# Itseez/opencv

Measured on AMD Instinct MI355X. Metric: Mpix/s per GPU (4K CV_8U Gaussian5x5) + achieved HBM GB/s vs roofline, 1/2/4/8 GPUs, higher is better.
Workload: dtype u8; 1 GPU; cv::GaussianBlur 5x5 sigma=0 BORDER_REFLECT_101 on 3840x2160 CV_8UC1, 9216 device-resident frames per GPU per step (152.9 GB of HBM: one pass = 18 launches of 512 frames); frames_per_gpu=9216, frames_per_launch=512, ranks=1, collective=none (1 GPU)

## Files before the change

### opencv_amd/csrc/smooth.hip

```cpp
#include "rt.h"
#include "gausskernel.h"
#include "seproll.h"
#include "seplong.h"
#include "sepmx.h"
#include <cstring>
#include <cstdlib>

using namespace mi355;

namespace {

struct FixedTaps { uint16_t kx[33]; uint16_t ky[33]; int nx, ny; };

__global__ __launch_bounds__(256) void k_sepfixed_generic(
    const uchar* __restrict__ src, size_t sstep, size_t sframe,
    uchar* __restrict__ dst, size_t dstep, size_t dframe,
    int W, int H, int cn, int mL, int mT, int mR, int mB, int border, FixedTaps t)
{
    const int b = blockIdx.x * 64 + (threadIdx.x & 63);
    const int y = blockIdx.y * 4 + (threadIdx.x >> 6);
    if (b >= W * cn || y >= H) return;
    src += (size_t)blockIdx.z * sframe;
    dst += (size_t)blockIdx.z * dframe;
    const int x = b / cn, c = b - x * cn;
    const int fullW = mL + W + mR, fullH = mT + H + mB;
    const int rx = t.nx / 2, ry = t.ny / 2;
    uint32_t acc = 0;
    for (int j = 0; j < t.ny; j++) {
        int yy = mi355_borderInterpolate(y + mT + j - ry, fullH, border);
        if (yy < 0) continue;
        const uchar* row = src + (ptrdiff_t)(yy - mT) * (ptrdiff_t)sstep;
        uint32_t h = 0;
        for (int i = 0; i < t.nx; i++) {
            int xx = mi355_borderInterpolate(x + mL + i - rx, fullW, border);
            if (xx < 0) continue;
            h += (uint32_t)t.kx[i] * row[(ptrdiff_t)(xx - mL) * cn + c];
        }
        h = h > 0xFFFFu ? 0xFFFFu : h;
        uint64_t a = (uint64_t)acc + (uint64_t)t.ky[j] * h;
        acc = a > 0xFFFFFFFFull ? 0xFFFFFFFFu : (uint32_t)a;
    }
    uint32_t r = (uint32_t)(((uint64_t)acc + 0x8000u) >> 16);
    dst[(size_t)y * dstep + b] = (uchar)(r > 255 ? 255 : r);
}

constexpr int floordiv2(int a) { return a >= 0 ? a / 2 : -((-a + 1) / 2); }
constexpr int mod2(int a) { return ((a % 2) + 2) % 2; }

template <int Q, int S, int HD>
__device__ __forceinline__ uint32_t pairAt(const uint32_t* E, const uint32_t* O, int k)
{
    constexpr int q2 = mod2(Q + S);
    constexpr int f = floordiv2(Q + S);
    const uint32_t* P = q2 ? O : E;
    if constexpr (mod2(f) == 0) {
        return P[k + f / 2 + HD];
    } else {
        constexpr int lo = floordiv2(f - 1) + 0;
        return __builtin_amdgcn_alignbit(P[k + lo + 1 + HD], P[k + lo + HD], 16);
    }
}

template <int HD> struct RawRow {
    uint4 m;
    uint32_t hl[HD];
    uint32_t hr[HD];
};

template <int KS, int CN> struct RollCfg {
    static constexpr int R = KS / 2;
    static constexpr int HB = R * CN;
    static constexpr int HD = (HB + 3) / 4;
};

template <int KS, int CN>
__device__ __forceinline__ void loadRow(RawRow<RollCfg<KS, CN>::HD>& r, const uchar* __restrict__ src, size_t sstep,
                                        int yy, int W, int H, int c, int nchunks, int lane, int border)
{
    constexpr int HD = RollCfg<KS, CN>::HD, HB = RollCfg<KS, CN>::HB;
    r.m = make_uint4(0, 0, 0, 0);
#pragma unroll
    for (int d = 0; d < HD; d++) { r.hl[d] = 0; r.hr[d] = 0; }
    const int ry = mi355_borderInterpolate(yy, H, border);
    if (ry < 0 || c >= nchunks) return;
    const uchar* row = src + (size_t)ry * sstep;
    r.m = *reinterpret_cast<const uint4*>(row + 16 * (size_t)c);
    if (lane == 0) {
        if (c > 0) {
#pragma unroll
            for (int d = 0; d < HD; d++) r.hl[d] = *reinterpret_cast<const uint32_t*>(row + 16 * (size_t)c - 4 * (HD - d));
        } else {
#pragma unroll
            for (int t = -HB; t < 0; t++) {
                const int px = (t - (CN - 1)) / CN;
                const int ch = t - px * CN;
                const int sp = mi355_borderInterpolate(px, W, border);
                const uint32_t v = sp < 0 ? 0u : row[sp * CN + ch];
                r.hl[(4 * HD + t) >> 2] |= v << (8 * ((4 * HD + t) & 3));
            }
        }
    }
    if (c == nchunks - 1) {
#pragma unroll
        for (int t = 0; t < HB; t++) {
            const int px = W + t / CN, ch = t % CN;
            const int sp = mi355_borderInterpolate(px, W, border);
            const uint32_t v = sp < 0 ? 0u : row[sp * CN + ch];
            r.hr[t >> 2] |= v << (8 * (t & 3));
        }
    } else if (lane == 63) {
#pragma unroll
        for (int d = 0; d < HD; d++) r.hr[d] = *reinterpret_cast<const uint32_t*>(row + 16 * (size_t)c + 16 + 4 * d);
    }
}

template <int KS, int CN>
__device__ __forceinline__ void hfilter(uint32_t (&Hrow)[8], const RawRow<RollCfg<KS, CN>::HD>& r, int c, int nchunks, int lane)
{
    constexpr int HD = RollCfg<KS, CN>::HD;
    constexpr int NW = 4 + 2 * HD;
    uint32_t X[NW];
    const uint32_t mv[4] = {r.m.x, r.m.y, r.m.z, r.m.w};
#pragma unroll
    for (int d = 0; d < HD; d++) {
        uint32_t l = __shfl_up(mv[4 - HD + d], 1);
        uint32_t rr = __shfl_down(mv[d], 1);
        X[d] = (lane == 0) ? r.hl[d] : l;
        X[HD + 4 + d] = (lane == 63 || c == nchunks - 1) ? r.hr[d] : rr;
    }
#pragma unroll
    for (int d = 0; d < 4; d++) X[HD + d] = mv[d];
    uint32_t E[NW], O[NW];
#pragma unroll
    for (int d = 0; d < NW; d++) {
        E[d] = __builtin_amdgcn_perm(0u, X[d], 0x0c020c00u);
        O[d] = __builtin_amdgcn_perm(0u, X[d], 0x0c030c01u);
    }
#pragma unroll
    for (int k = 0; k < 4; k++) {
        if constexpr (KS == 5) {
            {   uint32_t a = pairAt<0, -2 * CN, HD>(E, O, k) + pairAt<0, 2 * CN, HD>(E, O, k);
                uint32_t b = pairAt<0, -CN, HD>(E, O, k) + pairAt<0, CN, HD>(E, O, k);
                uint32_t m = pairAt<0, 0, HD>(E, O, k);
                Hrow[k] = a + (b << 2) + (m << 1) + (m << 2); }
            {   uint32_t a = pairAt<1, -2 * CN, HD>(E, O, k) + pairAt<1, 2 * CN, HD>(E, O, k);
                uint32_t b = pairAt<1, -CN, HD>(E, O, k) + pairAt<1, CN, HD>(E, O, k);
                uint32_t m = pairAt<1, 0, HD>(E, O, k);
                Hrow[4 + k] = a + (b << 2) + (m << 1) + (m << 2); }
        } else {
            Hrow[k]     = pairAt<0, -CN, HD>(E, O, k) + pairAt<0, CN, HD>(E, O, k) + (pairAt<0, 0, HD>(E, O, k) << 1);
            Hrow[4 + k] = pairAt<1, -CN, HD>(E, O, k) + pairAt<1, CN, HD>(E, O, k) + (pairAt<1, 0, HD>(E, O, k) << 1);
        }
    }
}

template <int KS, int CN>
__global__ __launch_bounds__(256) void k_binomial_roll(
    const uchar* __restrict__ src, size_t sstep, size_t sframe,
    uchar* __restrict__ dst, size_t dstep, size_t dframe,
    int W, int H, int nchunks, int segRows, int border)
{
    constexpr int R = KS / 2, HD = RollCfg<KS, CN>::HD;
    const int lane = threadIdx.x & 63;
    const int c = (blockIdx.x * 4 + (threadIdx.x >> 6)) * 64 + lane;
    const int y0 = blockIdx.y * segRows;
    const int y1 = min(H, y0 + segRows);
    src += (size_t)blockIdx.z * sframe;
    dst += (size_t)blockIdx.z * dframe;
    const bool active = c < nchunks;

    uint32_t Hw[KS][8];
    {
        RawRow<HD> pre[KS - 1];
#pragma unroll
        for (int i = 0; i < KS - 1; i++) loadRow<KS, CN>(pre[i], src, sstep, y0 - R + i, W, H, c, nchunks, lane, border);
#pragma unroll
        for (int i = 0; i < KS - 1; i++) hfilter<KS, CN>(Hw[i], pre[i], c, nchunks, lane);
    }
    for (int y = y0; y < y1; y += KS) {
        RawRow<HD> raw[KS];
#pragma unroll
        for (int u = 0; u < KS; u++)
            if (y + u < y1) loadRow<KS, CN>(raw[u], src, sstep, y + u + R, W, H, c, nchunks, lane, border);
#pragma unroll
        for (int u = 0; u < KS; u++) {
            if (y + u < y1) {
                hfilter<KS, CN>(Hw[(KS - 1 + u) % KS], raw[u], c, nchunks, lane);
                uint32_t o[4];
                if constexpr (KS == 5) {
                    const uint32_t* h0 = Hw[(u + 0) % 5]; const uint32_t* h1 = Hw[(u + 1) % 5];
                    const uint32_t* h2 = Hw[(u + 2) % 5]; const uint32_t* h3 = Hw[(u + 3) % 5];
                    const uint32_t* h4 = Hw[(u + 4) % 5];
                    uint32_t v[8];
#pragma unroll
                    for (int i = 0; i < 8; i++) {
                        const uint32_t b4 = lshlAdd(h1[i] + h3[i] + h2[i], 2, 0x00800080u);
                        v[i] = h0[i] + h4[i] + lshlAdd(h2[i], 1, b4);
                    }
#pragma unroll
                    for (int k = 0; k < 4; k++) o[k] = __builtin_amdgcn_perm(v[4 + k], v[k], 0x07030501u);
                } else {
                    const uint32_t* h0 = Hw[(u + 0) % 3]; const uint32_t* h1 = Hw[(u + 1) % 3]; const uint32_t* h2 = Hw[(u + 2) % 3];
#pragma unroll
                    for (int k = 0; k < 4; k++) {
                        uint32_t ve = ((h0[k] + h2[k] + (h1[k] << 1) + 0x00080008u) >> 4) & 0x00FF00FFu;
                        uint32_t vo = ((h0[4 + k] + h2[4 + k] + (h1[4 + k] << 1) + 0x00080008u) >> 4) & 0x00FF00FFu;
                        o[k] = ve | (vo << 8);
                    }
                }
                if (active)
                    *reinterpret_cast<uint4*>(dst + (size_t)(y + u) * dstep + 16 * (size_t)c) = make_uint4(o[0], o[1], o[2], o[3]);
            }
        }
    }
}

template <int HD> struct RawRow2 {
    uint4 m;
    uint32_t side[HD];
};

template <int HD> struct EdgeSel {
    uint32_t la[HD], lb[HD], lc[HD];
    uint32_t ra[HD], rb[HD], rc[HD];
};

__device__ __forceinline__ void selSetByte(uint32_t& a, uint32_t& b, uint32_t& c, int j, int idx )
{
    const uint32_t sh = 8u * (uint32_t)j, clr = ~(0xffu << sh);
    uint32_t va = 0x0cu, vb = 0x0cu, vc = 0x0cu;
    if (idx >= 8)      { vb = (uint32_t)(idx - 8); vc = 4u + (uint32_t)j; }
    else if (idx >= 0) { va = (uint32_t)idx;       vc = (uint32_t)j; }
    a = (a & clr) | (va << sh); b = (b & clr) | (vb << sh); c = (c & clr) | (vc << sh);
}

__device__ __forceinline__ uint32_t gather16(const uint4& m, uint32_t a, uint32_t b, uint32_t c)
{
    const uint32_t t1 = __builtin_amdgcn_perm(m.y, m.x, a);
    const uint32_t t2 = __builtin_amdgcn_perm(m.w, m.z, b);
    return __builtin_amdgcn_perm(t2, t1, c);
}

template <int KS, int CN, bool NTL = false>
__device__ __forceinline__ void issueRow(RawRow2<RollCfg<KS, CN>::HD>& r, const uchar* __restrict__ row, int mainOff, int sideOff)
{
    constexpr int HD = RollCfg<KS, CN>::HD;
    if constexpr (NTL) {
        typedef uint32_t u32x4 __attribute__((ext_vector_type(4)));
        u32x4 v = __builtin_nontemporal_load(reinterpret_cast<const u32x4*>(row + mainOff));
        r.m = make_uint4(v.x, v.y, v.z, v.w);
    } else
    r.m = *reinterpret_cast<const uint4*>(row + mainOff);
#pragma unroll
    for (int d = 0; d < HD; d++) r.side[d] = *reinterpret_cast<const uint32_t*>(row + sideOff + 4 * d);
}

template <int KS, int CN, bool EB = true>
__device__ __forceinline__ void hfilter2(uint32_t (&Hrow)[8], const RawRow2<RollCfg<KS, CN>::HD>& r,
                                         bool hasFirst, bool hasLast, bool isLastChunk, const EdgeSel<RollCfg<KS, CN>::HD>& es)
{
    constexpr int HD = RollCfg<KS, CN>::HD;
    constexpr int NW = 4 + 2 * HD;
    uint32_t X[NW];
    const uint32_t mv[4] = {r.m.x, r.m.y, r.m.z, r.m.w};
    uint32_t hl[HD], hr[HD];
#pragma unroll
    for (int d = 0; d < HD; d++) { hl[d] = r.side[d]; hr[d] = r.side[d]; }
    if (hasFirst) {
#pragma unroll
        for (int d = 0; d < HD; d++) { hl[d] = gather16(r.m, es.la[d], es.lb[d], es.lc[d]); if constexpr (EB) asm volatile("" : "+v"(hl[d])); }
    }
    uint32_t hb[HD];
#pragma unroll
    for (int d = 0; d < HD; d++) hb[d] = 0;
    if (hasLast) {
#pragma unroll
        for (int d = 0; d < HD; d++) { hb[d] = gather16(r.m, es.ra[d], es.rb[d], es.rc[d]); if constexpr (EB) asm volatile("" : "+v"(hb[d])); }
    }
#pragma unroll
    for (int d = 0; d < HD; d++) {
        X[d] = __builtin_amdgcn_update_dpp(hl[d], mv[4 - HD + d], 0x138, 0xf, 0xf, false);
        uint32_t rr = __builtin_amdgcn_update_dpp(hr[d], mv[d], 0x130, 0xf, 0xf, false);
        if (hasLast) { rr = isLastChunk ? hb[d] : rr; if constexpr (EB) asm volatile("" : "+v"(rr)); }
        X[HD + 4 + d] = rr;
    }
#pragma unroll
    for (int d = 0; d < 4; d++) X[HD + d] = mv[d];
    uint32_t E[NW], O[NW];
#pragma unroll
    for (int d = 0; d < NW; d++) {
        E[d] = __builtin_amdgcn_perm(0u, X[d], 0x0c020c00u);
        O[d] = __builtin_amdgcn_perm(0u, X[d], 0x0c030c01u);
    }
#pragma unroll
    for (int k = 0; k < 4; k++) {
        if constexpr (KS == 5) {
            {   uint32_t a = pairAt<0, -2 * CN, HD>(E, O, k) + pairAt<0, 2 * CN, HD>(E, O, k);
                uint32_t b = pairAt<0, -CN, HD>(E, O, k) + pairAt<0, CN, HD>(E, O, k);
                uint32_t m = pairAt<0, 0, HD>(E, O, k);
                Hrow[k] = a + (b << 2) + (m << 1) + (m << 2); }
            {   uint32_t a = pairAt<1, -2 * CN, HD>(E, O, k) + pairAt<1, 2 * CN, HD>(E, O, k);
                uint32_t b = pairAt<1, -CN, HD>(E, O, k) + pairAt<1, CN, HD>(E, O, k);
                uint32_t m = pairAt<1, 0, HD>(E, O, k);
                Hrow[4 + k] = a + (b << 2) + (m << 1) + (m << 2); }
        } else {
            Hrow[k]     = pairAt<0, -CN, HD>(E, O, k) + pairAt<0, CN, HD>(E, O, k) + (pairAt<0, 0, HD>(E, O, k) << 1);
            Hrow[4 + k] = pairAt<1, -CN, HD>(E, O, k) + pairAt<1, CN, HD>(E, O, k) + (pairAt<1, 0, HD>(E, O, k) << 1);
        }
    }
}

template <int KS, int CN, bool NT, bool NTL, int WPS, bool EB = true>
__global__ __launch_bounds__(256, WPS) void k_binomial_roll2(
    const uchar* __restrict__ src, size_t sstep, size_t sframe,
    uchar* __restrict__ dst, size_t dstep, size_t dframe,
    int W, int H, int nchunks, int nstrips, int segRows, int nseg, int nframes, int border, int alt)
{
    constexpr int R = KS / 2, HD = RollCfg<KS, CN>::HD, HB = RollCfg<KS, CN>::HB;
    const int lane = threadIdx.x & 63;
    const int wid = __builtin_amdgcn_readfirstlane((int)(blockIdx.x * 4 + (threadIdx.x >> 6)));
    const int strip = wid % nstrips;
    const int t0 = wid / nstrips;
    int seg = t0 % nseg;
    const int frame = t0 / nseg;
    if (frame >= nframes) return;
    int up = 0;
    if (alt) {
        const int G = 1 << alt, span = 8 * G;
        const int g = seg / span, j = seg - g * span;
        if ((g + 1) * span <= nseg) seg = g * span + G * (j & 7) + (j >> 3);
        else if (alt > 1) {
            const int base = g * span, t = seg - base, g2 = t >> 4, j2 = t & 15;
            if (base + (g2 << 4) + 16 <= nseg) seg = base + (g2 << 4) + 2 * (j2 & 7) + (j2 >> 3);
        }
        up = seg & 1;
    }
    const int c = strip * 64 + lane;
    const int y0 = seg * segRows;
    const int y1 = min(H, y0 + segRows);
    src += (size_t)frame * sframe;
    dst += (size_t)frame * dframe;
    const bool active = c < nchunks;
    const bool hasFirst = strip == 0, hasLast = strip == nstrips - 1;
    const bool isLastChunk = c == nchunks - 1;
    const int ce = active ? c : nchunks - 1;
    const int mainOff = 16 * ce;
    const int c0 = strip * 64;
    const int leftOff = c0 > 0 ? 16 * c0 - 4 * HD : 0;
    const int rightOff = c0 + 64 < nchunks ? 16 * (c0 + 64) : 16 * (nchunks - 1);
    const int sideOff = lane < 32 ? leftOff : rightOff;

    EdgeSel<HD> es;
#pragma unroll
    for (int d = 0; d < HD; d++) { es.la[d] = es.lb[d] = es.lc[d] = es.ra[d] = es.rb[d] = es.rc[d] = 0x0c0c0c0cu; }
    if (hasFirst) {
#pragma unroll
        for (int t = 0; t < HB; t++) {
            const int bt = t - HB;
            const int px = (bt - (CN - 1)) / CN;
            const int sp = mi355_borderInterpolate(px, W, border);
            const int pos = 4 * HD - HB + t;
            selSetByte(es.la[pos >> 2], es.lb[pos >> 2], es.lc[pos >> 2], pos & 3, sp < 0 ? -1 : sp * CN + (bt - px * CN));
        }
    }
    if (hasLast) {
#pragma unroll
        for (int t = 0; t < HB; t++) {
            const int sp = mi355_borderInterpolate(W + t / CN, W, border);
            selSetByte(es.ra[t >> 2], es.rb[t >> 2], es.rc[t >> 2], t & 3, sp < 0 ? -1 : sp * CN + (t % CN) - 16 * (nchunks - 1));
        }
    }
    int rowBelow[R], rowAbove[R];
#pragma unroll
    for (int i = 0; i < R; i++) { rowBelow[i] = mi355_borderInterpolate(H + i, H, border); rowAbove[i] = mi355_borderInterpolate(-1 - i, H, border); }
    const int nrows = y1 - y0;
    auto gy = [&](int j) -> int { return up ? y1 - 1 - j : y0 + j; };
    auto rowIdx = [&](int g) -> int {
        int ry = g;
#pragma unroll
        for (int i = 0; i < R; i++) { ry = (g == H + i) ? rowBelow[i] : ry; ry = (g == -1 - i) ? rowAbove[i] : ry; }
        return ry;
    };

    uint32_t Hw[KS][8];
#pragma unroll
    for (int i = 0; i < KS - 1; i++) {
        const int ry = rowIdx(gy(min(i - R, nrows - 1 + R)));
        if (ry < 0) {
#pragma unroll
            for (int j = 0; j < 8; j++) Hw[i][j] = 0;
        } else {
            RawRow2<HD> pre;
            issueRow<KS, CN>(pre, src + (size_t)ry * sstep, mainOff, sideOff);
            hfilter2<KS, CN, EB>(Hw[i], pre, hasFirst, hasLast, isLastChunk, es);
        }
    }
    RawRow2<HD> raw[KS];
    int rvalid[KS];
#pragma unroll
    for (int u = 0; u < KS; u++) {
        const int ry = rowIdx(gy(min(u + R, nrows - 1 + R)));
        rvalid[u] = ry >= 0;
        issueRow<KS, CN, NTL>(raw[u], src + (size_t)max(ry, 0) * sstep, mainOff, sideOff);
    }
    for (int y = 0; y < nrows; y += KS) {
#pragma unroll
        for (int u = 0; u < KS; u++) {
            if (y + u < nrows) {
                uint32_t (&Hn)[8] = Hw[(KS - 1 + u) % KS];
                if (rvalid[u]) hfilter2<KS, CN, EB>(Hn, raw[u], hasFirst, hasLast, isLastChunk, es);
                else {
#pragma unroll
                    for (int j = 0; j < 8; j++) Hn[j] = 0;
                }
                {
                    const int ry = rowIdx(gy(min(y + u + KS + R, nrows - 1 + R)));
                    rvalid[u] = ry >= 0;
                    issueRow<KS, CN, NTL>(raw[u], src + (size_t)max(ry, 0) * sstep, mainOff, sideOff);
                }
                uint32_t o[4];
                if constexpr (KS == 5) {
                    const uint32_t* h0 = Hw[(u + 0) % 5]; const uint32_t* h1 = Hw[(u + 1) % 5];
                    const uint32_t* h2 = Hw[(u + 2) % 5]; const uint32_t* h3 = Hw[(u + 3) % 5];
                    const uint32_t* h4 = Hw[(u + 4) % 5];
                    uint32_t v[8];
#pragma unroll
                    for (int i = 0; i < 8; i++) {
                        if constexpr (EB) {
                            const uint32_t b4 = lshlAdd(h1[i] + h3[i] + h2[i], 2, 0x00800080u);
                            v[i] = h0[i] + h4[i] + lshlAdd(h2[i], 1, b4);
                        } else
                            v[i] = (h0[i] + h4[i]) + ((h1[i] + h3[i]) << 2) + (h2[i] << 1) + (h2[i] << 2) + 0x00800080u;
                    }
#pragma unroll
                    for (int k = 0; k < 4; k++) o[k] = __builtin_amdgcn_perm(v[4 + k], v[k], 0x07030501u);
                } else {
                    const uint32_t* h0 = Hw[(u + 0) % 3]; const uint32_t* h1 = Hw[(u + 1) % 3]; const uint32_t* h2 = Hw[(u + 2) % 3];
#pragma unroll
                    for (int k = 0; k < 4; k++) {
                        uint32_t ve = ((h0[k] + h2[k] + (h1[k] << 1) + 0x00080008u) >> 4) & 0x00FF00FFu;
                        uint32_t vo = ((h0[4 + k] + h2[4 + k] + (h1[4 + k] << 1) + 0x00080008u) >> 4) & 0x00FF00FFu;
                        o[k] = ve | (vo << 8);
                    }
                }
                if (active) {
                    typedef uint32_t u32x4 __attribute__((ext_vector_type(4)));
                    u32x4 ov = {o[0], o[1], o[2], o[3]};
                    u32x4* dp = reinterpret_cast<u32x4*>(dst + (size_t)gy(y + u) * dstep + 16 * (size_t)c);
                    if constexpr (NT) __builtin_nontemporal_store(ov, dp);
                    else *dp = ov;
                }
            }
        }
    }
}

template <bool NT>
__global__ __launch_bounds__(256) void k_copy16(const uint4* __restrict__ s, uint4* __restrict__ d, size_t n16, int perThread)
{
    typedef uint32_t u32x4 __attribute__((ext_vector_type(4)));
    size_t base = ((size_t)blockIdx.x * perThread) * 256 + threadIdx.x;
#pragma unroll 4
    for (int i = 0; i < perThread; i++) {
        size_t j = base + (size_t)i * 256;
        if (j < n16) {
            uint4 v = s[j];
            u32x4 ov = {v.x, v.y, v.z, v.w};
            if constexpr (NT) __builtin_nontemporal_store(ov, reinterpret_cast<u32x4*>(d + j));
            else d[j] = v;
        }
    }
}

template <int UNROLL>
__global__ __launch_bounds__(256) void k_copy_colwalk(const uchar* __restrict__ src, uchar* __restrict__ dst, size_t step, size_t frame,
                                                      int H, int nchunks, int nstrips, int segRows, int nseg, int nframes)
{
    const int lane = threadIdx.x & 63;
    const int wid = __builtin_amdgcn_readfirstlane((int)(blockIdx.x * 4 + (threadIdx.x >> 6)));
    const int strip = wid % nstrips, t0 = wid / nstrips, seg = t0 % nseg, fr = t0 / nseg;
    if (fr >= nframes) return;
    const int c = strip * 64 + lane;
    if (c >= nchunks) return;
    const int y0 = seg * segRows, y1 = min(H, y0 + segRows);
    const uchar* s = src + (size_t)fr * frame + 16 * (size_t)c;
    uchar* d = dst + (size_t)fr * frame + 16 * (size_t)c;
    for (int y = y0; y < y1; y += UNROLL) {
        uint4 v[UNROLL];
#pragma unroll
        for (int u = 0; u < UNROLL; u++) v[u] = *reinterpret_cast<const uint4*>(s + (size_t)min(y + u, y1 - 1) * step);
#pragma unroll
        for (int u = 0; u < UNROLL; u++) if (y + u < y1) *reinterpret_cast<uint4*>(d + (size_t)(y + u) * step) = v[u];
    }
}


bool aligned16(const void* p, size_t step) { return (((uintptr_t)p | step) & 15) == 0; }

int envInt(const char* n, int d) { const char* v = getenv(n); return v ? atoi(v) : d; }

int& tuneSeg() { static int v = envInt("MI355CV_GAUSS_SEG", 0); return v; }
int& tuneVariant() { static int v = envInt("MI355CV_GAUSS_VARIANT", 3); return v; }

int& tuneAlt() { static int v = envInt("MI355CV_GAUSS_ALT", 1); return v; }
int& tuneLaunchWaves() { static int v = envInt("MI355CV_GAUSS_LAUNCH_WAVES", 393216); return v; }

template <int KS, int CN>
void launchRoll2(const uchar* s, size_t ss, size_t sf, uchar* d, size_t ds, size_t df, int nframes, int W, int H, int border, hipStream_t st, int nt)
{
    const int nchunks = W * CN / 16;
    const int nstrips = divUp(nchunks, 64);
    int seg = tuneSeg();
    if (seg <= 0) {
        long long per = (long long)nstrips * nframes;
        long long wantSeg = (2048 + per - 1) / per;
        seg = (int)((H + wantSeg - 1) / wantSeg);
        const int best = 16;
        if (seg > best) seg = best;
        if (seg < KS) seg = KS;
    }
    if (seg > H) seg = H;
    const int nseg = divUp(H, seg);
    const long long perFrame = (long long)nstrips * nseg;
    long long chunk = tuneLaunchWaves() > 0 ? (tuneLaunchWaves() + perFrame - 1) / perFrame : nframes;
    if (chunk < 1) chunk = 1;
    if (chunk > nframes) chunk = nframes;
    const int nlaunch = (int)((nframes + chunk - 1) / chunk);
    noteKernel("k_binomial_roll2<%d,%d,%s,false,%d,%s> grid=%u x256 seg=%d rows alt=%d, %d launch(es) of <= %lld frames", KS, CN, nt >= 1 ? "true" : "false", nt == 3 ? 6 : 4,
               nt == 2 ? "false" : "true", (unsigned)((perFrame * chunk + 3) / 4), seg, tuneAlt(), nlaunch, chunk);
    for (long long f0 = 0; f0 < nframes; f0 += chunk) {
        const int nf = (int)(nframes - f0 < chunk ? nframes - f0 : chunk);
        const uchar* sp = s + (size_t)f0 * sf;
        uchar* dp = d + (size_t)f0 * df;
        dim3 grid((unsigned)((perFrame * nf + 3) / 4));
        if (nt == 3)      hipLaunchKernelGGL((k_binomial_roll2<KS, CN, true, false, 6>), grid, dim3(256), 0, st, sp, ss, sf, dp, ds, df, W, H, nchunks, nstrips, seg, nseg, nf, border, tuneAlt());
        else if (nt == 2) hipLaunchKernelGGL((k_binomial_roll2<KS, CN, true, false, 4, false>), grid, dim3(256), 0, st, sp, ss, sf, dp, ds, df, W, H, nchunks, nstrips, seg, nseg, nf, border, tuneAlt());
        else if (nt == 1) hipLaunchKernelGGL((k_binomial_roll2<KS, CN, true, false, 4>), grid, dim3(256), 0, st, sp, ss, sf, dp, ds, df, W, H, nchunks, nstrips, seg, nseg, nf, border, tuneAlt());
        else              hipLaunchKernelGGL((k_binomial_roll2<KS, CN, false, false, 4>), grid, dim3(256), 0, st, sp, ss, sf, dp, ds, df, W, H, nchunks, nstrips, seg, nseg, nf, border, tuneAlt());
    }
}

template <int KS, int CN>
void launchRoll(const uchar* s, size_t ss, size_t sf, uchar* d, size_t ds, size_t df, int nframes, int W, int H, int border, hipStream_t st)
{
    const int nchunks = W * CN / 16;
    const int gx = divUp(nchunks, 256);
    const int segEnv = tuneSeg();
    int seg;
    if (segEnv > 0) seg = segEnv;
    else {
        long long stripsWaves = (long long)divUp(nchunks, 64) * nframes;
        long long wantSeg = (16384 + stripsWaves - 1) / stripsWaves;
        if (wantSeg < 1) wantSeg = 1;
        seg = (int)((H + wantSeg - 1) / wantSeg);
        if (seg < 4 * KS) seg = 4 * KS;
    }
    seg = divUp(seg, KS) * KS;
    if (seg > H) seg = divUp(H, KS) * KS;
    dim3 grid(gx, divUp(H, seg), nframes);
    hipLaunchKernelGGL((k_binomial_roll<KS, CN>), grid, dim3(256), 0, st, s, ss, sf, d, ds, df, W, H, nchunks, seg, border);
}

bool rollEligible(const uchar* s, size_t ss, size_t sf, const uchar* d, size_t ds, size_t df, int W, int H, int cn, int ks)
{
    if (ks != 3 && ks != 5) return false;
    if (cn < 1 || cn > 4) return false;
    if (!aligned16(s, ss) || !aligned16(d, ds) || (sf & 15) || (df & 15)) return false;
    if ((W * cn) % 16 != 0) return false;
    if (H < 1) return false;
    return true;
}

static int sepmxMinTaps()
{
    static const int v = std::getenv("MI355CV_SEPMX_MIN_TAPS") ? atoi(std::getenv("MI355CV_SEPMX_MIN_TAPS")) : 7;
    return v;
}

int runSmooth(const char* entry, const uchar* src, size_t sstep, size_t sframe, uchar* dst, size_t dstep, size_t dframe,
              int nframes, int W, int H, int cn, int mL, int mT, int mR, int mB,
              const uint16_t* kx, int nx, const uint16_t* ky, int ny, int border, bool binomial)
{
    if (disabled()) return mi355::declined(__func__, __LINE__, "disabled()");
    if (W <= 0 || H <= 0 || nframes <= 0 || cn < 1 || cn > 4) return mi355::declined(__func__, __LINE__, "W <= 0 || H <= 0 || nframes <= 0 || cn < 1 || cn > 4");
    if (nx < 1 || ny < 1 || nx > lim::GAUSS8U_MAX_KSIZE || ny > lim::GAUSS8U_MAX_KSIZE || !(nx & 1) || !(ny & 1)) return mi355::declined(__func__, __LINE__, "nx < 1 || ny < 1 || nx or ny > lim::GAUSS8U_MAX_KSIZE || !(nx & 1) || !(ny & 1)");
    if (border < 0 || border > B_REFLECT_101) return mi355::declined(__func__, __LINE__, "border < 0 || border > B_REFLECT_101");
    Stager stg;
    if (!ensureDevice()) return mi355::declined(__func__, __LINE__, "!ensureDevice()");
    const bool hostSrc = !isDevicePtr(src);
    if (hostSrc && (size_t)W * H < minPixels()) return mi355::declined(__func__, __LINE__, "hostSrc && (size_t)W * H < minPixels()");
    if (!hostSrc && src == dst) return mi355::declined(__func__, __LINE__, "!hostSrc && src == dst");

    size_t dss = 0, dds = 0;
    const size_t rowB = (size_t)W * cn;
    const uchar* dsrc; uchar* ddst;
    if (nframes == 1) {
        const uchar* top = src - (ptrdiff_t)mT * (ptrdiff_t)sstep - (ptrdiff_t)mL * cn;
        const uchar* dtop = stg.in(top, sstep, (size_t)(mL + W + mR) * cn, mT + H + mB, &dss);
        if (!dtop) return mi355::declined(__func__, __LINE__, "!dtop");
        dsrc = dtop + (size_t)mT * dss + (size_t)mL * cn;
        ddst = stg.out(dst, dstep, rowB, H, &dds);
        if (!ddst) return mi355::declined(__func__, __LINE__, "!ddst");
    } else {
        if (hostSrc || !isDevicePtr(dst)) return setError(MI355CV_NOT_IMPLEMENTED, "%s: batch entry needs device-resident frames", entry);
        dsrc = src; ddst = dst; dss = sstep; dds = dstep;
    }
    hipStream_t st = stream();
    const bool noMargins = !(mL | mT | mR | mB);
    if (binomial && noMargins && rollEligible(dsrc, dss, sframe, ddst, dds, dframe, W, H, cn, nx) && nx == ny) {
#define ROLL(KS_, CN_) do { if (tuneVariant() <= 1 || border == B_WRAP || W <= KS_ / 2) launchRoll<KS_, CN_>(dsrc, dss, sframe, ddst, dds, dframe, nframes, W, H, border, st); \
                            else launchRoll2<KS_, CN_>(dsrc, dss, sframe, ddst, dds, dframe, nframes, W, H, border, st, tuneVariant() - 2); } while (0)
        if (nx == 5) { switch (cn) { case 1: ROLL(5, 1); break; case 2: ROLL(5, 2); break; case 3: ROLL(5, 3); break; default: ROLL(5, 4); } }
        else         { switch (cn) { case 1: ROLL(3, 1); break; case 2: ROLL(3, 2); break; case 3: ROLL(3, 3); break; default: ROLL(3, 4); } }
#undef ROLL
    } else if (std::getenv("MI355CV_SMOOTH_GENERIC") == nullptr && std::max(nx, ny) >= sepmxMinTaps() && !(std::getenv("MI355CV_SEPMX") && std::getenv("MI355CV_SEPMX")[0] == '0') &&
               sepmxRun(stg, dsrc, dss, sframe, ddst, dds, dframe, nframes, W, H, cn, mL + W + mR, mT + H + mB, mL, mT, border, kx, nx, nx / 2, ky, ny, ny / 2, st)) {
    } else if (noMargins && std::getenv("MI355CV_SMOOTH_GENERIC") == nullptr &&
               seprollFixedSmooth(dsrc, dss, sframe, ddst, dds, dframe, nframes, W, H, cn, kx, nx, ky, ny, border, st)) {
    } else if (!noMargins && nframes == 1 && std::getenv("MI355CV_SMOOTH_GENERIC") == nullptr && [&] {
                   const Roi roi = {mL + W + mR, mT + H + mB, mL, mT};
                   return seprollFixedSmooth(dsrc, dss, 0, ddst, dds, 0, 1, W, H, cn, kx, nx, ky, ny, border, st, &roi); }()) {
    } else if (std::getenv("MI355CV_SMOOTH_GENERIC") == nullptr && std::max(nx, ny) < sepmxMinTaps() && !(std::getenv("MI355CV_SEPMX") && std::getenv("MI355CV_SEPMX")[0] == '0') &&
               sepmxRun(stg, dsrc, dss, sframe, ddst, dds, dframe, nframes, W, H, cn, mL + W + mR, mT + H + mB, mL, mT, border, kx, nx, nx / 2, ky, ny, ny / 2, st)) {
    } else if (std::getenv("MI355CV_SMOOTH_GENERIC") == nullptr && [&] {
                   unsigned sx = 0, sy = 0;
                   for (int i = 0; i < nx; i++) sx += kx[i];
                   for (int i = 0; i < ny; i++) sy += ky[i];
                   if (sx > 256 || sy > 256) return false;
                   std::vector<int> ix(kx, kx + nx), iy(ky, ky + ny);
                   const SepLongTaps t = {nullptr, nullptr, ix.data(), iy.data(), nx, ny, nx / 2, ny / 2, 3, 0, 0.f, 0};
                   return seplongRun(stg, dsrc, dss, sframe, ddst, dds, dframe, nframes, W, H, cn, MI355CV_8U, MI355CV_8U, mL + W + mR, mT + H + mB, mL, mT, border, t, st); }()) {
    } else {
        if (nx > 33 || ny > 33) return mi355::declined(__func__, __LINE__, "Q8.8 taps that sum beyond 256 with more than 33 of them");
        FixedTaps t;
        t.nx = nx; t.ny = ny;
        for (int i = 0; i < 33; i++) { t.kx[i] = i < nx ? kx[i] : 0; t.ky[i] = i < ny ? ky[i] : 0; }
        dim3 grid(divUp(W * cn, 64), divUp(H, 4), nframes);
        hipLaunchKernelGGL(k_sepfixed_generic, grid, dim3(256), 0, st, dsrc, dss, sframe, ddst, dds, dframe,
                           W, H, cn, mL, mT, mR, mB, border, t);
    }
    return stg.finish(entry);
}

template <int K>
__global__ __launch_bounds__(256) void k_binom16_direct(const uchar* __restrict__ parent, size_t sstep, uchar* __restrict__ dst, size_t dstep, int W, int H, int cn,
                                                        int mL, int mT, int fullW, int fullH, int border)
{
    constexpr int R = K / 2, SH = K == 3 ? 2 : K == 5 ? 4 : K == 7 ? 6 : 8;
    constexpr uint32_t TAP[9] = {K == 3 ? 1u : K == 5 ? 1u : K == 7 ? 2u : 4u, K == 3 ? 2u : K == 5 ? 4u : K == 7 ? 7u : 13u, K == 3 ? 1u : K == 5 ? 6u : K == 7 ? 14u : 30u,
                                 K == 5 ? 4u : K == 7 ? 18u : 51u, K == 5 ? 1u : K == 7 ? 14u : 60u, K == 7 ? 7u : 51u, K == 7 ? 2u : 30u, 13u, 4u};
    const int e = blockIdx.x * 64 + (threadIdx.x & 63), y = blockIdx.y * 4 + (threadIdx.x >> 6);
    if (e >= W * cn || y >= H) return;
    const int x = e / cn, c = e - x * cn;
    int xs[K];
#pragma unroll
    for (int i = 0; i < K; i++) { const int q = mi355_borderInterpolate(x + mL + i - R, fullW, border); xs[i] = q < 0 ? -1 : q * cn + c; }
    uint32_t acc = 0;
#pragma unroll
    for (int j = 0; j < K; j++) {
        const int q = mi355_borderInterpolate(y + mT + j - R, fullH, border);
        if (q < 0) continue;
        const unsigned short* row = reinterpret_cast<const unsigned short*>(parent + (size_t)q * sstep);
        uint32_t h = 0;
#pragma unroll
        for (int i = 0; i < K; i++) h += xs[i] < 0 ? 0u : TAP[i] * (uint32_t)row[xs[i]];
        acc += TAP[j] * h;
    }
    reinterpret_cast<unsigned short*>(dst + (size_t)y * dstep)[e] = (unsigned short)((acc + (1u << (2 * SH - 1))) >> (2 * SH));
}

int runBinom16(const char* entry, const uchar* src, size_t sstep, uchar* dst, size_t dstep, int W, int H, int cn, int mL, int mT, int mR, int mB, int ksize, int border)
{
    if (disabled() || W <= 0 || H <= 0 || cn < 1 || cn > 4 || (ksize != 3 && ksize != 5 && ksize != 7 && ksize != 9) || border < 0 || border > B_REFLECT_101 ||
        mL < 0 || mT < 0 || mR < 0 || mB < 0 || ((sstep | dstep | (uintptr_t)src | (uintptr_t)dst) & 1))
        return mi355::declined(__func__, __LINE__, "disabled() || W <= 0 || H <= 0 || cn < 1 || cn > 4 || ksize not in {3, 5, 7, 9} || border outside CONSTANT .. REFLECT_101 || negative margins || odd pointers / steps");
    Stager stg;
    if (!ensureDevice()) return mi355::declined(__func__, __LINE__, "!ensureDevice()");
    const bool hostSrc = !isDevicePtr(src);
    if (hostSrc && (size_t)W * H < minPixels()) return mi355::declined(__func__, __LINE__, "hostSrc && (size_t)W * H < minPixels()");
    if (!hostSrc && src == dst) return mi355::declined(__func__, __LINE__, "!hostSrc && src == dst");
    size_t dss = 0, dds = 0;
    const size_t esz = (size_t)cn * 2;
    const uchar* top = src - (ptrdiff_t)mT * (ptrdiff_t)sstep - (ptrdiff_t)mL * (ptrdiff_t)esz;
    const uchar* dtop = stg.in(top, sstep, (size_t)(mL + W + mR) * esz, mT + H + mB, &dss);
    if (!dtop) return mi355::declined(__func__, __LINE__, "!dtop");
    const uchar* dsrc = dtop + (size_t)mT * dss + (size_t)mL * esz;
    uchar* ddst = stg.out(dst, dstep, (size_t)W * esz, H, &dds);
    if (!ddst) return mi355::declined(__func__, __LINE__, "!ddst");
    const Roi roi = {mL + W + mR, mT + H + mB, mL, mT};
    if (cn == 1 && (ksize == 3 || ksize == 5) && border != B_WRAP &&
        seprollBinom16(dsrc, dss, 0, ddst, dds, 0, 1, W, H, ksize, border, stream(), (mL | mT | mR | mB) ? &roi : nullptr))
        return stg.finish(entry);
    dim3 grid(divUp(W * cn, 64), divUp(H, 4));
#define B16(K_) hipLaunchKernelGGL(k_binom16_direct<K_>, grid, dim3(256), 0, stream(), dtop, dss, ddst, dds, W, H, cn, mL, mT, mL + W + mR, mT + H + mB, border)
    if (ksize == 3) B16(3); else if (ksize == 5) B16(5); else if (ksize == 7) B16(7); else B16(9);
#undef B16
    noteKernel("k_binom16_direct<%d> grid=%ux%u x256 cn=%d border=%d", ksize, grid.x, grid.y, cn, border);
    return stg.finish(entry);
}

const uint16_t kBinom1[1] = {256};
const uint16_t kBinom3[3] = {64, 128, 64};
const uint16_t kBinom5[5] = {16, 64, 96, 64, 16};
const uint16_t kBinom7[7] = {8, 28, 56, 72, 56, 28, 8};
const uint16_t kBinom9[9] = {4, 13, 30, 51, 60, 51, 30, 13, 4};

const uint16_t* binomTaps(size_t k)
{
    switch (k) { case 1: return kBinom1; case 3: return kBinom3; case 5: return kBinom5; case 7: return kBinom7; case 9: return kBinom9; }
    return nullptr;
}

}

extern "C" {

MI355CV_API int mi355cv_gaussianBlurBinomial(const uchar* src_data, size_t src_step, uchar* dst_data, size_t dst_step,
        int width, int height, int depth, int cn, size_t margin_left, size_t margin_top, size_t margin_right,
        size_t margin_bottom, size_t ksize, int border_type)
{
    mi355::EntryGuard entry_(__func__);
    if (depth == MI355CV_16U)
        return runBinom16("gaussianBlurBinomial", src_data, src_step, dst_data, dst_step, width, height, cn, (int)margin_left, (int)margin_top, (int)margin_right,
                                 (int)margin_bottom, (int)ksize, border_type & ~MI355CV_BORDER_ISOLATED);
    if (depth != MI355CV_8U) return mi355::declined(__func__, __LINE__, "depth != MI355CV_8U");
    const uint16_t* k = binomTaps(ksize);
    if (!k) return mi355::declined(__func__, __LINE__, "!k");
    return runSmooth("gaussianBlurBinomial", src_data, src_step, 0, dst_data, dst_step, 0, 1, width, height, cn,
                     (int)margin_left, (int)margin_top, (int)margin_right, (int)margin_bottom,
                     k, (int)ksize, k, (int)ksize, border_type & ~MI355CV_BORDER_ISOLATED, true);
}

static int gaussBatchFromHost(const uchar* src, size_t sstep, size_t sframe, uchar* dst, size_t dstep, size_t dframe, int nframes, int W, int H, int cn,
                              const uint16_t* k, int ks, int border)
{
    const HostBatch hb = {src, sstep, sframe, (size_t)W * cn, H, dst, dstep, dframe, (size_t)W * cn, H, nframes};
    return runHostBatch("gaussianBlurBinomialBatch", hb, [&](const uchar* s, size_t ss, size_t sf, uchar* d, size_t ds, size_t df, int nf) {
        return runSmooth("gaussianBlurBinomialBatch", s, ss, nf > 1 ? sf : 0, d, ds, nf > 1 ? df : 0, nf, W, H, cn, 0, 0, 0, 0, k, ks, k, ks, border, true);
    });
}

MI355CV_API int mi355cv_gaussianBlurBinomialBatch(const uchar* src_data, size_t src_step, size_t src_frame_stride,
        uchar* dst_data, size_t dst_step, size_t dst_frame_stride, int nframes,
        int width, int height, int depth, int cn, size_t ksize, int border_type)
{
    mi355::EntryGuard entry_(__func__);
    if (depth != MI355CV_8U) return mi355::declined(__func__, __LINE__, "depth != MI355CV_8U");
    const uint16_t* k = binomTaps(ksize);
    if (!k) return mi355::declined(__func__, __LINE__, "!k");
    if (nframes > 1 && width > 0 && height > 0 && cn >= 1 && cn <= 4 && hostBatchEligible(src_data, dst_data, nframes))
        return gaussBatchFromHost(src_data, src_step, src_frame_stride, dst_data, dst_step, dst_frame_stride, nframes, width, height, cn, k, (int)ksize,
                                  border_type & ~MI355CV_BORDER_ISOLATED);
    if (nframes == 1)
        return runSmooth("gaussianBlurBinomialBatch", src_data, src_step, 0, dst_data, dst_step, 0, 1, width, height, cn,
                         0, 0, 0, 0, k, (int)ksize, k, (int)ksize, border_type & ~MI355CV_BORDER_ISOLATED, true);
    return runSmooth("gaussianBlurBinomialBatch", src_data, src_step, src_frame_stride, dst_data, dst_step, dst_frame_stride,
                     nframes, width, height, cn, 0, 0, 0, 0, k, (int)ksize, k, (int)ksize,
                     border_type & ~MI355CV_BORDER_ISOLATED, true);
}

MI355CV_API int mi355cv_gaussianBlur(const uchar* src_data, size_t src_step, uchar* dst_data, size_t dst_step,
        int width, int height, int depth, int cn, size_t margin_left, size_t margin_top, size_t margin_right,
        size_t margin_bottom, size_t ksize_width, size_t ksize_height, double sigmaX, double sigmaY, int border_type)
{
    mi355::EntryGuard entry_(__func__);
    if (depth != MI355CV_8U) {
        if (depth != MI355CV_16U && depth != MI355CV_16S && depth != MI355CV_32F) return mi355::declined(__func__, __LINE__, "depth is none of 8U / 16U / 16S / 32F");
        const int n = (int)ksize_width, m = (int)ksize_height;
        if (n < 1 || m < 1 || n > lim::GAUSS_FLOAT_MAX_KSIZE || m > lim::GAUSS_FLOAT_MAX_KSIZE || !(n & 1) || !(m & 1)) return mi355::declined(__func__, __LINE__, "kernel size outside 1 .. lim::GAUSS_FLOAT_MAX_KSIZE or even");
        if (sigmaY <= 0) sigmaY = sigmaX;
        const double s1 = sigmaX > 0 ? sigmaX : 0, s2 = sigmaY > 0 ? sigmaY : 0;
        std::vector<double> dx, dy;
        if (!gaussianKernelBitExact(n, s1, dx)) return mi355::declined(__func__, __LINE__, "!gaussianKernelBitExact(n, s1, dx)");
        if (m == n && std::fabs(s1 - s2) < 2.220446049250313e-16) dy = dx;
        else if (!gaussianKernelBitExact(m, s2, dy)) return mi355::declined(__func__, __LINE__, "!gaussianKernelBitExact(m, s2, dy)");
        std::vector<float> fx(dx.begin(), dx.end()), fy(dy.begin(), dy.end());
        const int type = MI355CV_MAKETYPE(depth, cn);
        cvhalFilter2D* ctx = nullptr;
        int rc = mi355cv_sepFilterInit(&ctx, type, type, MI355CV_32F, reinterpret_cast<uchar*>(fx.data()), n, reinterpret_cast<uchar*>(fy.data()), m, -1, -1, 0.0, border_type);
        if (rc != MI355CV_OK) return rc;
        rc = mi355cv_sepFilter(ctx, const_cast<uchar*>(src_data), src_step, dst_data, dst_step, width, height, (int)(margin_left + (size_t)width + margin_right),
                               (int)(margin_top + (size_t)height + margin_bottom), (int)margin_left, (int)margin_top);
        (void)mi355cv_sepFilterFree(ctx);
        return rc;
    }
    if (margin_left | margin_top | margin_right | margin_bottom)
        return mi355::setError(MI355CV_NOT_IMPLEMENTED, "gaussianBlur: submatrix with real margins is the reference's sepFilter2D case");
    if (ksize_width > (size_t)lim::GAUSS8U_MAX_KSIZE || ksize_height > (size_t)lim::GAUSS8U_MAX_KSIZE) return mi355::declined(__func__, __LINE__, "ksize_width or ksize_height > lim::GAUSS8U_MAX_KSIZE");
    if (sigmaY <= 0) sigmaY = sigmaX;
    std::vector<int64_t> qx, qy;
    if (!gaussianKernelFixedQ((int)ksize_width, sigmaX > 0 ? sigmaX : 0, 8, qx)) return mi355::declined(__func__, __LINE__, "!gaussianKernelFixedQ((int)ksize_width, sigmaX > 0 ? sigmaX : 0, 8, qx)");
    if (!gaussianKernelFixedQ((int)ksize_height, sigmaY > 0 ? sigmaY : 0, 8, qy)) return mi355::declined(__func__, __LINE__, "!gaussianKernelFixedQ((int)ksize_height, sigmaY > 0 ? sigmaY : 0, 8, qy)");
    uint16_t kx[lim::GAUSS8U_MAX_KSIZE], ky[lim::GAUSS8U_MAX_KSIZE];
    for (size_t i = 0; i < ksize_width; i++) { if (qx[i] < 0 || qx[i] > 65535) return mi355::declined(__func__, __LINE__, "qx[i] < 0 || qx[i] > 65535"); kx[i] = (uint16_t)qx[i]; }
    for (size_t i = 0; i < ksize_height; i++) { if (qy[i] < 0 || qy[i] > 65535) return mi355::declined(__func__, __LINE__, "qy[i] < 0 || qy[i] > 65535"); ky[i] = (uint16_t)qy[i]; }
    bool binom = ksize_width == ksize_height && (ksize_width == 3 || ksize_width == 5);
    if (binom) {
        const uint16_t* b = binomTaps(ksize_width);
        for (size_t i = 0; i < ksize_width; i++) if (kx[i] != b[i] || ky[i] != b[i]) binom = false;
    }
    return runSmooth("gaussianBlur", src_data, src_step, 0, dst_data, dst_step, 0, 1, width, height, cn,
                     (int)margin_left, (int)margin_top, (int)margin_right, (int)margin_bottom,
                     kx, (int)ksize_width, ky, (int)ksize_height, border_type & ~MI355CV_BORDER_ISOLATED, binom);
}

MI355CV_API int mi355cv_gaussianBlurBatch(const uchar* src_data, size_t src_step, size_t src_frame_stride, uchar* dst_data, size_t dst_step, size_t dst_frame_stride,
        int nframes, int width, int height, int depth, int cn, size_t ksize_width, size_t ksize_height, double sigmaX, double sigmaY, int border_type)
{
    mi355::EntryGuard entry_(__func__);
    if (depth != MI355CV_8U) return mi355::declined(__func__, __LINE__, "depth != MI355CV_8U");
    if (nframes < 1 || !(ksize_width & 1) || !(ksize_height & 1) || ksize_width > (size_t)lim::GAUSS8U_MAX_KSIZE || ksize_height > (size_t)lim::GAUSS8U_MAX_KSIZE)
        return mi355::declined(__func__, __LINE__, "nframes < 1 || even kernel size || ksize > lim::GAUSS8U_MAX_KSIZE");
    if (sigmaY <= 0) sigmaY = sigmaX;
    std::vector<int64_t> qx, qy;
    if (!gaussianKernelFixedQ((int)ksize_width, sigmaX > 0 ? sigmaX : 0, 8, qx) || !gaussianKernelFixedQ((int)ksize_height, sigmaY > 0 ? sigmaY : 0, 8, qy))
        return mi355::declined(__func__, __LINE__, "!gaussianKernelFixedQ");
    uint16_t kx[lim::GAUSS8U_MAX_KSIZE], ky[lim::GAUSS8U_MAX_KSIZE];
    for (size_t i = 0; i < ksize_width; i++) { if (qx[i] < 0 || qx[i] > 65535) return mi355::declined(__func__, __LINE__, "qx[i] < 0 || qx[i] > 65535"); kx[i] = (uint16_t)qx[i]; }
    for (size_t i = 0; i < ksize_height; i++) { if (qy[i] < 0 || qy[i] > 65535) return mi355::declined(__func__, __LINE__, "qy[i] < 0 || qy[i] > 65535"); ky[i] = (uint16_t)qy[i]; }
    bool binom = ksize_width == ksize_height && (ksize_width == 3 || ksize_width == 5);
    if (binom) {
        const uint16_t* b = binomTaps(ksize_width);
        for (size_t i = 0; i < ksize_width; i++) if (kx[i] != b[i] || ky[i] != b[i]) binom = false;
    }
    return runSmooth("gaussianBlurBatch", src_data, src_step, nframes > 1 ? src_frame_stride : 0, dst_data, dst_step, nframes > 1 ? dst_frame_stride : 0, nframes, width, height, cn,
                     0, 0, 0, 0, kx, (int)ksize_width, ky, (int)ksize_height, border_type & ~MI355CV_BORDER_ISOLATED, binom);
}

MI355CV_API int mi355cv_setParam(const char* key, int value)
{
    mi355::EntryGuard entry_(__func__);
    if (!key) return -1;
    if (!strcmp(key, "gauss_seg")) { tuneSeg() = value; return 0; }
    if (!strcmp(key, "gauss_variant")) { tuneVariant() = value; return 0; }
    if (!strcmp(key, "gauss_alt")) { tuneAlt() = value; return 0; }
    if (!strcmp(key, "gauss_launch_waves")) { tuneLaunchWaves() = value; return 0; }
    return -1;
}

MI355CV_API int mi355cv_copyProbe(const void* src, void* dst, size_t bytes, int perThread, int nt)
{
    mi355::EntryGuard entry_(__func__);
    if (!ensureDevice() || (bytes & 15) || perThread < 1) return mi355::declined(__func__, __LINE__, "!ensureDevice() || (bytes & 15) || perThread < 1");
    size_t n16 = bytes / 16;
    size_t blocks = (n16 + (size_t)256 * perThread - 1) / ((size_t)256 * perThread);
    if (nt) hipLaunchKernelGGL((k_copy16<true>), dim3((unsigned)blocks), dim3(256), 0, stream(), (const uint4*)src, (uint4*)dst, n16, perThread);
    else    hipLaunchKernelGGL((k_copy16<false>), dim3((unsigned)blocks), dim3(256), 0, stream(), (const uint4*)src, (uint4*)dst, n16, perThread);
    if (hipGetLastError() != hipSuccess) return MI355CV_ERROR_UNKNOWN;
    if (!asyncMode()) (void)hipStreamSynchronize(stream());
    return MI355CV_OK;
}

MI355CV_API int mi355cv_copyProbeColwalk(const void* src, void* dst, int W, int H, int nframes, int segRows, int unroll)
{
    mi355::EntryGuard entry_(__func__);
    if (!ensureDevice() || (W & 15)) return mi355::declined(__func__, __LINE__, "!ensureDevice() || (W & 15)");
    const int nchunks = W / 16, nstrips = divUp(nchunks, 64), nseg = divUp(H, segRows);
    const long long items = (long long)nstrips * nseg * nframes;
    dim3 grid((unsigned)((items + 3) / 4));
    const uchar* s = (const uchar*)src; uchar* d = (uchar*)dst;
    if (unroll == 1) hipLaunchKernelGGL((k_copy_colwalk<1>), grid, dim3(256), 0, stream(), s, d, (size_t)W, (size_t)W * H, H, nchunks, nstrips, segRows, nseg, nframes);
    else if (unroll == 2) hipLaunchKernelGGL((k_copy_colwalk<2>), grid, dim3(256), 0, stream(), s, d, (size_t)W, (size_t)W * H, H, nchunks, nstrips, segRows, nseg, nframes);
    else if (unroll == 5) hipLaunchKernelGGL((k_copy_colwalk<5>), grid, dim3(256), 0, stream(), s, d, (size_t)W, (size_t)W * H, H, nchunks, nstrips, segRows, nseg, nframes);
    else hipLaunchKernelGGL((k_copy_colwalk<10>), grid, dim3(256), 0, stream(), s, d, (size_t)W, (size_t)W * H, H, nchunks, nstrips, segRows, nseg, nframes);
    if (hipGetLastError() != hipSuccess) return MI355CV_ERROR_UNKNOWN;
    if (!asyncMode()) (void)hipStreamSynchronize(stream());
    return MI355CV_OK;
}

MI355CV_API int mi355cv_getGaussianKernelQ(int n, double sigma, int fractionBits, int64_t* taps)
{
    mi355::EntryGuard entry_(__func__);
    std::vector<int64_t> q;
    if (!gaussianKernelFixedQ(n, sigma, fractionBits, q)) return mi355::declined(__func__, __LINE__, "!gaussianKernelFixedQ(n, sigma, fractionBits, q)");
    for (int i = 0; i < n; i++) taps[i] = q[i];
    return MI355CV_OK;
}

MI355CV_API int mi355cv_getGaussianKernel(int n, double sigma, double* taps)
{
    mi355::EntryGuard entry_(__func__);
    std::vector<double> k;
    if (!gaussianKernelBitExact(n, sigma, k)) return mi355::declined(__func__, __LINE__, "!gaussianKernelBitExact(n, sigma, k)");
    for (int i = 0; i < n; i++) taps[i] = k[i];
    return MI355CV_OK;
}

MI355CV_API int mi355cv_sepSmoothFixedU8(const uchar* src_data, size_t src_step, uchar* dst_data, size_t dst_step,
        int width, int height, int cn, size_t margin_left, size_t margin_top, size_t margin_right, size_t margin_bottom,
        const uint16_t* kx, int kxlen, const uint16_t* ky, int kylen, int border_type)
{
    mi355::EntryGuard entry_(__func__);
    if (!kx || !ky) return mi355::declined(__func__, __LINE__, "!kx || !ky");
    bool binom = kxlen == kylen && (kxlen == 3 || kxlen == 5);
    if (binom) {
        const uint16_t* b = binomTaps(kxlen);
        for (int i = 0; i < kxlen; i++) if (kx[i] != b[i] || ky[i] != b[i]) binom = false;
    }
    return runSmooth("sepSmoothFixedU8", src_data, src_step, 0, dst_data, dst_step, 0, 1, width, height, cn,
                     (int)margin_left, (int)margin_top, (int)margin_right, (int)margin_bottom,
                     kx, kxlen, ky, kylen, border_type & ~MI355CV_BORDER_ISOLATED, binom);
}

}
```

Measured before the change: 2.965 million Mpix/s.

## Add RING prologue variant issuing all halo row loads before filtering

```diff
diff --git a/opencv_amd/csrc/smooth.hip b/opencv_amd/csrc/smooth.hip
--- a/opencv_amd/csrc/smooth.hip
+++ b/opencv_amd/csrc/smooth.hip
@@ -310,7 +310,7 @@
     }
 }
 
-template <int KS, int CN, bool NT, bool NTL, int WPS, bool EB = true>
+template <int KS, int CN, bool NT, bool NTL, int WPS, bool EB = true, bool RING = false>
 __global__ __launch_bounds__(256, WPS) void k_binomial_roll2(
     const uchar* __restrict__ src, size_t sstep, size_t sframe,
     uchar* __restrict__ dst, size_t dstep, size_t dframe,
@@ -383,72 +383,114 @@
     };
 
     uint32_t Hw[KS][8];
-#pragma unroll
-    for (int i = 0; i < KS - 1; i++) {
-        const int ry = rowIdx(gy(min(i - R, nrows - 1 + R)));
-        if (ry < 0) {
-#pragma unroll
-            for (int j = 0; j < 8; j++) Hw[i][j] = 0;
-        } else {
-            RawRow2<HD> pre;
-            issueRow<KS, CN>(pre, src + (size_t)ry * sstep, mainOff, sideOff);
-            hfilter2<KS, CN, EB>(Hw[i], pre, hasFirst, hasLast, isLastChunk, es);
-        }
-    }
     RawRow2<HD> raw[KS];
     int rvalid[KS];
-#pragma unroll
-    for (int u = 0; u < KS; u++) {
-        const int ry = rowIdx(gy(min(u + R, nrows - 1 + R)));
+    auto consume = [&](int u) __attribute__((always_inline)) {
+        uint32_t (&Hn)[8] = Hw[(KS - 1 + u) % KS];
+        if (rvalid[u]) hfilter2<KS, CN, EB>(Hn, raw[u], hasFirst, hasLast, isLastChunk, es);
+        else {
+#pragma unroll
+            for (int j = 0; j < 8; j++) Hn[j] = 0;
+        }
+    };
+    auto refill = [&](int u, int j) __attribute__((always_inline)) {
+        const int ry = rowIdx(gy(min(j, nrows - 1 + R)));
         rvalid[u] = ry >= 0;
         issueRow<KS, CN, NTL>(raw[u], src + (size_t)max(ry, 0) * sstep, mainOff, sideOff);
-    }
-    for (int y = 0; y < nrows; y += KS) {
+    };
+    auto emit = [&](int u, int j) __attribute__((always_inline)) {
+        uint32_t o[4];
+        if constexpr (KS == 5) {
+            const uint32_t* h0 = Hw[(u + 0) % 5]; const uint32_t* h1 = Hw[(u + 1) % 5];
+            const uint32_t* h2 = Hw[(u + 2) % 5]; const uint32_t* h3 = Hw[(u + 3) % 5];
+            const uint32_t* h4 = Hw[(u + 4) % 5];
+            uint32_t v[8];
+#pragma unroll
+            for (int i = 0; i < 8; i++) {
+                if constexpr (EB) {
+                    const uint32_t b4 = lshlAdd(h1[i] + h3[i] + h2[i], 2, 0x00800080u);
+                    v[i] = h0[i] + h4[i] + lshlAdd(h2[i], 1, b4);
+                } else
+                    v[i] = (h0[i] + h4[i]) + ((h1[i] + h3[i]) << 2) + (h2[i] << 1) + (h2[i] << 2) + 0x00800080u;
+            }
+#pragma unroll
+            for (int k = 0; k < 4; k++) o[k] = __builtin_amdgcn_perm(v[4 + k], v[k], 0x07030501u);
+        } else {
+            const uint32_t* h0 = Hw[(u + 0) % 3]; const uint32_t* h1 = Hw[(u + 1) % 3]; const uint32_t* h2 = Hw[(u + 2) % 3];
+#pragma unroll
+            for (int k = 0; k < 4; k++) {
+                uint32_t ve = ((h0[k] + h2[k] + (h1[k] << 1) + 0x00080008u) >> 4) & 0x00FF00FFu;
+                uint32_t vo = ((h0[4 + k] + h2[4 + k] + (h1[4 + k] << 1) + 0x00080008u) >> 4) & 0x00FF00FFu;
+                o[k] = ve | (vo << 8);
+            }
+        }
+        if (active) {
+            typedef uint32_t u32x4 __attribute__((ext_vector_type(4)));
+            u32x4 ov = {o[0], o[1], o[2], o[3]};
+            u32x4* dp = reinterpret_cast<u32x4*>(dst + (size_t)gy(j) * dstep + 16 * (size_t)c);
+            if constexpr (NT) __builtin_nontemporal_store(ov, dp);
+            else *dp = ov;
+        }
+    };
+    if constexpr (RING) {
+        RawRow2<HD> pre[KS - 1];
+        int pvalid[KS - 1];
+#pragma unroll
+        for (int i = 0; i < KS - 1; i++) {
+            const int ry = rowIdx(gy(min(i - R, nrows - 1 + R)));
+            pvalid[i] = ry >= 0;
+            issueRow<KS, CN>(pre[i], src + (size_t)max(ry, 0) * sstep, mainOff, sideOff);
+            __builtin_amdgcn_sched_barrier(0);
+        }
 #pragma unroll
         for (int u = 0; u < KS; u++) {
+            refill(u, u + R);
+            __builtin_amdgcn_sched_barrier(0);
+        }
+#pragma unroll
+        for (int i = 0; i < KS - 1; i++) {
+            hfilter2<KS, CN, EB>(Hw[i], pre[i], hasFirst, hasLast, isLastChunk, es);
+#pragma unroll
+            for (int j = 0; j < 8; j++) Hw[i][j] = pvalid[i] ? Hw[i][j] : 0u;
+        }
+        int y = 0;
+        for (; y + KS <= nrows; y += KS) {
+#pragma unroll
+            for (int u = 0; u < KS; u++) {
+                consume(u);
+                refill(u, y + u + KS + R);
+                emit(u, y + u);
+            }
+        }
+#pragma unroll
+        for (int u = 0; u < KS - 1; u++) {
             if (y + u < nrows) {
-                uint32_t (&Hn)[8] = Hw[(KS - 1 + u) % KS];
-                if (rvalid[u]) hfilter2<KS, CN, EB>(Hn, raw[u], hasFirst, hasLast, isLastChunk, es);
-                else {
-#pragma unroll
-                    for (int j = 0; j < 8; j++) Hn[j] = 0;
-                }
-                {
-                    const int ry = rowIdx(gy(min(y + u + KS + R, nrows - 1 + R)));
-                    rvalid[u] = ry >= 0;
-                    issueRow<KS, CN, NTL>(raw[u], src + (size_t)max(ry, 0) * sstep, mainOff, sideOff);
-                }
-                uint32_t o[4];
-                if constexpr (KS == 5) {
-                    const uint32_t* h0 = Hw[(u + 0) % 5]; const uint32_t* h1 = Hw[(u + 1) % 5];
-                    const uint32_t* h2 = Hw[(u + 2) % 5]; const uint32_t* h3 = Hw[(u + 3) % 5];
-                    const uint32_t* h4 = Hw[(u + 4) % 5];
-                    uint32_t v[8];
-#pragma unroll
-                    for (int i = 0; i < 8; i++) {
-                        if constexpr (EB) {
-                            const uint32_t b4 = lshlAdd(h1[i] + h3[i] + h2[i], 2, 0x00800080u);
-                            v[i] = h0[i] + h4[i] + lshlAdd(h2[i], 1, b4);
-                        } else
-                            v[i] = (h0[i] + h4[i]) + ((h1[i] + h3[i]) << 2) + (h2[i] << 1) + (h2[i] << 2) + 0x00800080u;
-                    }
-#pragma unroll
-                    for (int k = 0; k < 4; k++) o[k] = __builtin_amdgcn_perm(v[4 + k], v[k], 0x07030501u);
-                } else {
-                    const uint32_t* h0 = Hw[(u + 0) % 3]; const uint32_t* h1 = Hw[(u + 1) % 3]; const uint32_t* h2 = Hw[(u + 2) % 3];
-#pragma unroll
-                    for (int k = 0; k < 4; k++) {
-                        uint32_t ve = ((h0[k] + h2[k] + (h1[k] << 1) + 0x00080008u) >> 4) & 0x00FF00FFu;
-                        uint32_t vo = ((h0[4 + k] + h2[4 + k] + (h1[4 + k] << 1) + 0x00080008u) >> 4) & 0x00FF00FFu;
-                        o[k] = ve | (vo << 8);
-                    }
-                }
-                if (active) {
-                    typedef uint32_t u32x4 __attribute__((ext_vector_type(4)));
-                    u32x4 ov = {o[0], o[1], o[2], o[3]};
-                    u32x4* dp = reinterpret_cast<u32x4*>(dst + (size_t)gy(y + u) * dstep + 16 * (size_t)c);
-                    if constexpr (NT) __builtin_nontemporal_store(ov, dp);
-                    else *dp = ov;
+                consume(u);
+                emit(u, y + u);
+            }
+        }
+    } else {
+#pragma unroll
+        for (int i = 0; i < KS - 1; i++) {
+            const int ry = rowIdx(gy(min(i - R, nrows - 1 + R)));
+            if (ry < 0) {
+#pragma unroll
+                for (int j = 0; j < 8; j++) Hw[i][j] = 0;
+            } else {
+                RawRow2<HD> pre;
+                issueRow<KS, CN>(pre, src + (size_t)ry * sstep, mainOff, sideOff);
+                hfilter2<KS, CN, EB>(Hw[i], pre, hasFirst, hasLast, isLastChunk, es);
+            }
+        }
+#pragma unroll
+        for (int u = 0; u < KS; u++) refill(u, u + R);
+        for (int y = 0; y < nrows; y += KS) {
+#pragma unroll
+            for (int u = 0; u < KS; u++) {
+                if (y + u < nrows) {
+                    consume(u);
+                    refill(u, y + u + KS + R);
+                    emit(u, y + u);
                 }
             }
         }
@@ -500,7 +542,8 @@
 int envInt(const char* n, int d) { const char* v = getenv(n); return v ? atoi(v) : d; }
 
 int& tuneSeg() { static int v = envInt("MI355CV_GAUSS_SEG", 0); return v; }
-int& tuneVariant() { static int v = envInt("MI355CV_GAUSS_VARIANT", 3); return v; }
+constexpr int kGaussVariantDefault = 6;
+int& tuneVariant() { static int v = envInt("MI355CV_GAUSS_VARIANT", kGaussVariantDefault); return v; }
 
 int& tuneAlt() { static int v = envInt("MI355CV_GAUSS_ALT", 1); return v; }
 int& tuneLaunchWaves() { static int v = envInt("MI355CV_GAUSS_LAUNCH_WAVES", 393216); return v; }
@@ -515,7 +558,7 @@
         long long per = (long long)nstrips * nframes;
         long long wantSeg = (2048 + per - 1) / per;
         seg = (int)((H + wantSeg - 1) / wantSeg);
-        const int best = 16;
+        const int best = (nt == 4 && CN == 1) ? 12 : 16;
         if (seg > best) seg = best;
         if (seg < KS) seg = KS;
     }
@@ -526,14 +569,15 @@
     if (chunk < 1) chunk = 1;
     if (chunk > nframes) chunk = nframes;
     const int nlaunch = (int)((nframes + chunk - 1) / chunk);
-    noteKernel("k_binomial_roll2<%d,%d,%s,false,%d,%s> grid=%u x256 seg=%d rows alt=%d, %d launch(es) of <= %lld frames", KS, CN, nt >= 1 ? "true" : "false", nt == 3 ? 6 : 4,
-               nt == 2 ? "false" : "true", (unsigned)((perFrame * chunk + 3) / 4), seg, tuneAlt(), nlaunch, chunk);
+    noteKernel("k_binomial_roll2<%d,%d,%s,false,%d,%s%s> grid=%u x256 seg=%d rows alt=%d, %d launch(es) of <= %lld frames", KS, CN, nt >= 1 ? "true" : "false", nt == 3 ? 6 : 4,
+               nt == 2 ? "false" : "true", nt == 4 ? ",true" : "", (unsigned)((perFrame * chunk + 3) / 4), seg, tuneAlt(), nlaunch, chunk);
     for (long long f0 = 0; f0 < nframes; f0 += chunk) {
         const int nf = (int)(nframes - f0 < chunk ? nframes - f0 : chunk);
         const uchar* sp = s + (size_t)f0 * sf;
         uchar* dp = d + (size_t)f0 * df;
         dim3 grid((unsigned)((perFrame * nf + 3) / 4));
-        if (nt == 3)      hipLaunchKernelGGL((k_binomial_roll2<KS, CN, true, false, 6>), grid, dim3(256), 0, st, sp, ss, sf, dp, ds, df, W, H, nchunks, nstrips, seg, nseg, nf, border, tuneAlt());
+        if (nt >= 4)      hipLaunchKernelGGL((k_binomial_roll2<KS, CN, true, false, 4, true, true>), grid, dim3(256), 0, st, sp, ss, sf, dp, ds, df, W, H, nchunks, nstrips, seg, nseg, nf, border, tuneAlt());
+        else if (nt == 3) hipLaunchKernelGGL((k_binomial_roll2<KS, CN, true, false, 6>), grid, dim3(256), 0, st, sp, ss, sf, dp, ds, df, W, H, nchunks, nstrips, seg, nseg, nf, border, tuneAlt());
         else if (nt == 2) hipLaunchKernelGGL((k_binomial_roll2<KS, CN, true, false, 4, false>), grid, dim3(256), 0, st, sp, ss, sf, dp, ds, df, W, H, nchunks, nstrips, seg, nseg, nf, border, tuneAlt());
         else if (nt == 1) hipLaunchKernelGGL((k_binomial_roll2<KS, CN, true, false, 4>), grid, dim3(256), 0, st, sp, ss, sf, dp, ds, df, W, H, nchunks, nstrips, seg, nseg, nf, border, tuneAlt());
         else              hipLaunchKernelGGL((k_binomial_roll2<KS, CN, false, false, 4>), grid, dim3(256), 0, st, sp, ss, sf, dp, ds, df, W, H, nchunks, nstrips, seg, nseg, nf, border, tuneAlt());
@@ -832,7 +876,7 @@
     mi355::EntryGuard entry_(__func__);
     if (!key) return -1;
     if (!strcmp(key, "gauss_seg")) { tuneSeg() = value; return 0; }
-    if (!strcmp(key, "gauss_variant")) { tuneVariant() = value; return 0; }
+    if (!strcmp(key, "gauss_variant")) { tuneVariant() = value > 0 ? value : kGaussVariantDefault; return 0; }
     if (!strcmp(key, "gauss_alt")) { tuneAlt() = value; return 0; }
     if (!strcmp(key, "gauss_launch_waves")) { tuneLaunchWaves() = value; return 0; }
     return -1;
```

Result: faster. 3.053 million Mpix/s, median of 6 (+3.0%).
